# MAGIC-SCAN/adipose_tissue-unet

Measured on AMD Instinct MI355X. Metric: 1024^2 tiles/sec (train), higher is better.
Workload: dtype bf16; 1 GPU; unet_bn L5 base64 1024x1024x3 bf16 B=4/GPU (BASELINE configs[2]); preset=unet_bn, levels=5, tile=1024, batch_per_gpu=4, global_batch=4, parallelism=dp1

## Files before the change

### adipose_tissue-unet_amd/csrc/conv_fwd_halo.hip

```cpp
#include <type_traits>

#include "conv_common.h"

namespace {

__device__ __attribute__((aligned(256))) uint4 halo_zero_page[64];

constexpr int PH = 8, PW = 32;
constexpr int HH = PH + 2, HW = PW + 2;
constexpr int HROWS = HH * HW;
constexpr int ROWB = 128;

__device__ __forceinline__ int hswz(int r) { return r & 7; }

#define LDS_BAR()                                             \
  do {                                                        \
    asm volatile("s_waitcnt lgkmcnt(0)" ::: "memory");        \
    __builtin_amdgcn_s_barrier();                             \
    asm volatile("" ::: "memory");                            \
  } while (0)

#define HALO_BAR()                         \
  do {                                     \
    asm volatile("" ::: "memory");         \
    __builtin_amdgcn_s_barrier();          \
    asm volatile("" ::: "memory");         \
  } while (0)

template <int WN, int KS, int TPS, int NHB>
constexpr int halo_lds() {
  constexpr int NTH = 4 * WN * KS * 64;
  constexpr int GH = (HROWS * 8 + NTH - 1) / NTH;
  return NHB * (GH * NTH / 8) * ROWB + 3 * TPS * WN * 64 * ROWB;
}

template <int WN, int KS, int TPS, int NHB, bool BNR>
__global__ __launch_bounds__(4 * WN * KS * 64, (halo_lds<WN, KS, TPS, NHB>() <= 81920 ? 2 : 1))
void igemm_fwd_halo_kernel(FwdArgs a) {
  constexpr int NTH = 4 * WN * KS * 64;
  constexpr int BN = WN * 64;
  constexpr int SPC = (9 + TPS - 1) / TPS;
  constexpr int GH = (HROWS * 8 + NTH - 1) / NTH;
  constexpr int HROWS_PAD = GH * NTH / 8;
  constexpr int HBUF = HROWS_PAD * ROWB;
  constexpr int GB1 = BN * 8 / NTH;
  static_assert(GB1 * NTH == BN * 8, "weight slot must split evenly");
  constexpr int GB = GB1 * TPS;
  constexpr int WTAP = BN * ROWB;
  constexpr int WSLOT = TPS * WTAP;
  constexpr int OFF_W = NHB * HBUF;
  constexpr int LT = BN + 4;
  constexpr int EPI = PH * PW * LT * 4;
  constexpr int SMEM = (OFF_W + 3 * WSLOT > EPI) ? OFF_W + 3 * WSLOT : EPI;
  __shared__ __attribute__((aligned(1024))) unsigned char smem[SMEM];

  const int tid = threadIdx.x, lane = tid & 63;
  const int wave = __builtin_amdgcn_readfirstlane(tid >> 6);
  const int wm = wave % 4, wn = (wave / 4) % WN, kh = wave / (4 * WN);
  const int tx_n = a.Wo / PW, ty_n = a.Ho / PH;
  const int lin = xcd_remap(blockIdx.x, a.nblocks);
  const int tn = lin % a.ntile_n;
  int rest = lin / a.ntile_n;
  const int px = rest % tx_n; rest /= tx_n;
  const int py = rest % ty_n;
  const int img = rest / ty_n;
  const int y0 = py * PH, x0 = px * PW, n0 = tn * BN;
  const int Cin_s = a.CAs + a.CBs;
  const int nchunk = Cin_s / 64, nsteps = nchunk * SPC;
  const int Wrows = (a.Nout + 63) / 64 * 64;
  const bf16* srcA = reinterpret_cast<const bf16*>(a.srcA);
  const bf16* srcB = reinterpret_cast<const bf16*>(a.srcB);

  int hoff[GH], hcol[GH];
#pragma unroll
  for (int i = 0; i < GH; ++i) {
    const int idx = i * NTH + tid;
    const int hr = idx >> 3, pos = idx & 7;
    hcol[i] = 8 * (pos ^ hswz(hr));
    const int gy = y0 - 1 + hr / HW, gx = x0 - 1 + hr % HW;
    hoff[i] = (hr < HROWS && gy >= 0 && gy < a.Hs && gx >= 0 && gx < a.Ws) ? (img * a.Hs + gy) * a.Ws + gx : -1;
  }
  const bf16* wp[GB1];
#pragma unroll
  for (int i = 0; i < GB1; ++i) {
    const int idx = i * NTH + tid;
    const int q = idx >> 3, pos = idx & 7;
    wp[i] = (n0 + q < Wrows) ? reinterpret_cast<const bf16*>(a.W) + (size_t)(n0 + q) * a.Kpad + 8 * (pos ^ swz(q))
                             : nullptr;
  }

  auto issue_halo = [&](int c, int buf) {
    const int ci = c * 64;
    const bf16* base = ci < a.CAs ? srcA + ci : srcB + (ci - a.CAs);
    const int cs = ci < a.CAs ? a.CAs : a.CBs;
    unsigned char* dst = smem + buf * HBUF + wave * 8 * ROWB;
#pragma unroll
    for (int i = 0; i < GH; ++i) {
      const void* p = hoff[i] >= 0 ? (const void*)(base + (size_t)hoff[i] * cs + hcol[i]) : (const void*)halo_zero_page;
      __builtin_amdgcn_global_load_lds(p, (lds_void*)(dst + i * (NTH / 8) * ROWB), 16, 0, 0);
    }
  };
  auto issue_w = [&](int s) {
    const int c = s / SPC, j = s - SPC * c;
#pragma unroll
    for (int u = 0; u < TPS; ++u) {
      const int t = j * TPS + u;
      const int k = t * Cin_s + c * 64;
      unsigned char* dst = smem + OFF_W + (s % 3) * WSLOT + u * WTAP + wave * 8 * ROWB;
#pragma unroll
      for (int i = 0; i < GB1; ++i) {
        const void* p = (wp[i] && t < 9) ? (const void*)(wp[i] + k) : (const void*)halo_zero_page;
        __builtin_amdgcn_global_load_lds(p, (lds_void*)(dst + i * (NTH / 8) * ROWB), 16, 0, 0);
      }
    }
  };

  f32x4 acc[4][4];
#pragma unroll
  for (int i = 0; i < 4; ++i)
#pragma unroll
    for (int j = 0; j < 4; ++j) acc[i][j] = f32x4{0.f, 0.f, 0.f, 0.f};

  const int r16 = lane & 15, h4 = lane >> 4;
  issue_halo(0, 0);
  issue_w(0);
  if (nsteps > 1) {
    issue_w(1);
    asm volatile("s_waitcnt vmcnt(%0)" ::"n"(GB) : "memory");
  } else {
    asm volatile("s_waitcnt vmcnt(0)" ::: "memory");
  }
  HALO_BAR();

  for (int s = 0; s < nsteps; ++s) {
    const int c = s / SPC, j = s - SPC * c;
    const bool nh = NHB == 2 && j == 0 && c + 1 < nchunk;
    if (nh) issue_halo(c + 1, (c + 1) & 1);
    const bool nw = s + 2 < nsteps;
    if (nw) issue_w(s + 2);
    const unsigned char* H = smem + (NHB == 2 ? (c & 1) : 0) * HBUF;
#pragma unroll
    for (int u = 0; u < TPS; ++u) {
    const int t = j * TPS + u;
    if (t >= 9) break;
    const int dy = t / 3, dx = t - 3 * dy;
    const unsigned char* Wt = smem + OFF_W + (s % 3) * WSLOT + u * WTAP;
#pragma unroll
    for (int kq = 0; kq < 2 / KS; ++kq) {
      const int ck = 4 * (KS == 2 ? kh : kq) + h4;
      bf16x8 fb[4], fa[4];
#pragma unroll
      for (int nf = 0; nf < 4; ++nf) {
        const int q = wn * 64 + nf * 16 + r16;
        fb[nf] = *reinterpret_cast<const bf16x8*>(Wt + q * ROWB + ((ck ^ swz(q)) << 4));
      }
#pragma unroll
      for (int mf = 0; mf < 4; ++mf) {
        const int prow = 2 * wm + (mf >> 1), pcol = (mf & 1) * 16 + r16;
        const int hr = (prow + dy) * HW + pcol + dx;
        fa[mf] = *reinterpret_cast<const bf16x8*>(H + hr * ROWB + ((ck ^ hswz(hr)) << 4));
      }
#pragma unroll
      for (int mf = 0; mf < 4; ++mf)
#pragma unroll
        for (int nf = 0; nf < 4; ++nf)
          acc[mf][nf] = __builtin_amdgcn_mfma_f32_16x16x32_bf16(fa[mf], fb[nf], acc[mf][nf], 0, 0, 0);
    }
    }
    if (nw) {
      if (nh) asm volatile("s_waitcnt vmcnt(%0)" ::"n"(GB + GH) : "memory");
      else asm volatile("s_waitcnt vmcnt(%0)" ::"n"(GB) : "memory");
    } else {
      asm volatile("s_waitcnt vmcnt(0)" ::: "memory");
    }
    HALO_BAR();
  }

  float* tile = reinterpret_cast<float*>(smem);
  const int col = lane & 15, rq = (lane >> 4) * 4;
#pragma unroll
  for (int part = 0; part < KS; ++part) {
    if (kh == part) {
#pragma unroll
      for (int mf = 0; mf < 4; ++mf)
#pragma unroll
        for (int nf = 0; nf < 4; ++nf)
#pragma unroll
          for (int r = 0; r < 4; ++r) {
            const int p = (2 * wm + (mf >> 1)) * PW + (mf & 1) * 16 + rq + r;
            float* e = tile + p * LT + wn * 64 + nf * 16 + col;
            *e = part == 0 ? acc[mf][nf][r] : *e + acc[mf][nf][r];
          }
    }
    ADP_LDS_BARRIER();
  }
  float bs[8], bq[8];
#pragma unroll
  for (int j = 0; j < 8; ++j) { bs[j] = 0.f; bq[j] = 0.f; }
  for (int pr = 0; pr < PH; ++pr) {
    const int m0 = (img * a.Ho + y0 + pr) * a.Wo + x0;
    if constexpr (BNR) epi_rows_bnr<NTH, BN>(a, tile + pr * PW * LT, PW, m0, n0, tid, bs, bq);
    else epi_rows<NTH, BN>(a, tile + pr * PW * LT, PW, m0, n0, tid, bs, bq);
  }
  if (a.bn_sum || a.bnr_z) epi_bn_flush<NTH, BN>(a, tile, n0, tid, bs, bq);
}

#ifndef HALOP_VALU_PER_MFMA
#define HALOP_VALU_PER_MFMA 8
#endif
template <int I, int N, typename F>
__device__ __forceinline__ void halop_static_for(F&& f) {
  if constexpr (I < N) {
    f(std::integral_constant<int, I>{});
    halop_static_for<I + 1, N>(f);
  }
}
template <bool BNR, int NCH, int BN, bool PIPE, int EPI_, bool WIDE = false, bool DYN = false, bool SWP = false>
__global__ __launch_bounds__(512, 1) void igemm_fwd_halop_kernel(FwdArgs a) {
  constexpr bool BNL = EPI_ == 6;
  constexpr int EPI = BNL ? 1 : EPI_;
  static_assert(!BNL || (!BNR && !DYN && !SWP && NCH == 1), "BN-on-load: one-chunk static-list forward launches");
  static_assert(!BNR || EPI == 0, "the BN-backward reduction launch stores the plain product");
  static_assert(EPI < 4 || !PIPE, "mask / addend quads, the dropout hash and two accumulator sets: registers");
  constexpr int NTH = 512, NF = BN / 16;
  constexpr int HCH = NCH * HROWS * 8;
  constexpr int GH = (HCH + NTH - 1) / NTH;
  static_assert(!BNL || GH <= 6, "BN-on-load: at most six halo chunks per thread");
  constexpr int HBUF = HCH * 16;
  constexpr int GW = 9 * NCH * BN * 8 / NTH;
  constexpr int WTAP = NCH * BN * ROWB;
  constexpr int OFF_W = HBUF, OFF_C = OFF_W + 9 * WTAP;
  constexpr int OFF_S = OFF_C + 5 * BN * 4 + 16;
  constexpr int SMEM = OFF_S + (BNL ? 2 * NCH * 64 * 4 : 0);
  static_assert(GW * NTH == 9 * NCH * BN * 8, "weights must split evenly");
  static_assert(SMEM <= 160 * 1024, "LDS");
  typedef __bf16 bf16x4 __attribute__((ext_vector_type(4)));
  typedef unsigned int v2u32_h __attribute__((ext_vector_type(2)));
  typedef unsigned int v4u32_h __attribute__((ext_vector_type(4)));
  __shared__ __attribute__((aligned(1024))) unsigned char smem[SMEM];

  const int tid = threadIdx.x, lane = tid & 63;
  const int wave = __builtin_amdgcn_readfirstlane(tid >> 6);
  prio_static<ADP_PRIO_FWD>(wave);
  const int tx_n = a.Wo / PW, ty_n = a.Ho / PH;
  const int T = a.nblocks, G = gridDim.x;
  const int lin = xcd_remap(blockIdx.x, G);
  constexpr bool dyn = DYN;
  const bool full = dyn && a.claim_full;
  const int nt = dyn ? 0 : (lin < T ? (T - lin + G - 1) / G : 0);
  if (!dyn && nt == 0) return;
  const int Wrows = (a.Nout + 63) / 64 * 64;
  const int NT = a.ntile_n;
  const int nh = lin % NT, n0 = BN * nh;
  const bool second = a.out_mode == 2 && n0 >= a.split_c;
  bf16* obase = reinterpret_cast<bf16*>(second ? a.out2 : a.out);
  const int ostride = second ? a.out2_stride : a.out_stride;
  const int ocol0 = second ? n0 - a.split_c : n0;
  const int nlim = a.out_mode == 2 && !second ? a.split_c : a.Nout;
  const int Cin_s = a.CAs + a.CBs;

  int* ring = reinterpret_cast<int*>(smem + OFF_C + 5 * BN * 4);
  const int npatch = T / NT;
  const int CH = dyn ? a.claim_chunk : 1, nsup = (npatch + CH - 1) / CH;
  auto sup_id = [&](int sidx) -> int {
    const int v = full ? claim_ring_read(ring + (sidx & 3))
                       : sidx < 2 ? lin / NT + sidx * (G / NT) : 2 * (G / NT) + claim_ring_read(ring + (sidx & 3));
    return v < nsup ? v : -1;
  };
  auto tile_id = [&](int k) -> int {
    if (!dyn) return k < nt ? lin / NT + k * (G / NT) : -1;
    const int v = sup_id(k / CH);
    const int t = v * CH + k % CH;
    return v >= 0 && t < npatch ? t : -1;
  };
  if (full) {
    if (tid == 0) {
      const int r = claim_next2(a.claim + nh);
      ring[0] = r;
      ring[1] = r + 1;
    }
    __syncthreads();
  }
  if (dyn && tile_id(0) < 0) {
    if (tid == 0) claim_block_done(a.claim, NT, G);
    return;
  }
  auto tile_origin = [&](int t, int& img, int& y0, int& x0) {
    const int px = t % tx_n, r = t / tx_n;
    y0 = (r % ty_n) * PH;
    img = r / ty_n;
    x0 = px * PW;
  };
  auto halo_src = [&](int img, int y0, int x0, int i) -> const uint4* {
    const int idx = i * NTH + tid;
    const int cc = NCH == 1 ? 0 : (idx >= HROWS * 8 ? 1 : 0), hr = (idx - cc * HROWS * 8) >> 3;
    const int hy = hr / HW, hx = hr - hy * HW;
    const int gy = y0 + hy - 1, gx = x0 + hx - 1, us = a.up >> 1;
    const bool ok = (i < GH - 1 || idx < HCH) && (unsigned)gy < (unsigned)(a.Hs << us) && (unsigned)gx < (unsigned)(a.Ws << us);
    if (!ok) return nullptr;
    const bool inA = cc * 64 < a.CAs;
    const bf16* src = reinterpret_cast<const bf16*>(inA ? a.srcA : a.srcB);
    const int cs = inA ? a.CAs : a.CBs;
    return reinterpret_cast<const uint4*>(src + (size_t)((img * a.Hs + (gy >> us)) * a.Ws + (gx >> us)) * cs +
                                          (inA ? cc * 64 : cc * 64 - a.CAs) + 8 * ((tid & 7) ^ hswz(hr)));
  };

  const float* sS = reinterpret_cast<const float*>(smem + OFF_S);
  const bool act_w = BNL && n0 == 0 && a.act_out != nullptr && !(ADP_DBG(a) & 4096);
  const __amdgpu_buffer_rsrc_t rsA = __builtin_amdgcn_make_buffer_rsrc(
      a.act_out, 0, act_w ? a.Nimg * a.Hs * a.Ws * a.CAs * 2 : 0, 0x00020000);
  auto bnl = [&](uint4 v, int img, int y0, int x0, int i) -> uint4 {
    const int idx = i * NTH + tid;
    const int cc = NCH == 1 ? 0 : (idx >= HROWS * 8 ? 1 : 0), hr = (idx - cc * HROWS * 8) >> 3;
    const int hy = hr / HW, hx = hr - hy * HW;
    const int gy = y0 + hy - 1, gx = x0 + hx - 1;
    const bool inimg = (unsigned)gy < (unsigned)a.Hs && (unsigned)gx < (unsigned)a.Ws;
    const int c0 = cc * 64 + 8 * ((tid & 7) ^ hswz(hr));
    Grp<bf16> g;
    g.v = v;
    bf16* e = reinterpret_cast<bf16*>(&g.v);
#pragma unroll
    for (int hv = 0; hv < 2; ++hv) {
      const float4 q = *reinterpret_cast<const float4*>(sS + c0 + 4 * hv);
      const float4 r = *reinterpret_cast<const float4*>(sS + NCH * 64 + c0 + 4 * hv);
      e[4 * hv + 0] = (bf16)fmaxf(fmaf((float)e[4 * hv + 0], q.x, r.x), 0.f);
      e[4 * hv + 1] = (bf16)fmaxf(fmaf((float)e[4 * hv + 1], q.y, r.y), 0.f);
      e[4 * hv + 2] = (bf16)fmaxf(fmaf((float)e[4 * hv + 2], q.z, r.z), 0.f);
      e[4 * hv + 3] = (bf16)fmaxf(fmaf((float)e[4 * hv + 3], q.w, r.w), 0.f);
    }
    const bool wr = inimg && hy >= 1 && hy <= PH && hx >= 1 && hx <= PW;
    const unsigned off = wr ? (unsigned)((((img * a.Hs + gy) * a.Ws + gx) * a.CAs + c0) * 2) : 0x80000000u;
    if (act_w) __builtin_amdgcn_raw_buffer_store_b128(__builtin_bit_cast(v4u32_h, g.v), rsA, off, 0, 0);
    return inimg ? g.v : v;
  };

#pragma unroll
  for (int i = 0; i < GW; ++i) {
    const int idx = i * NTH + tid;
    const int tc = idx / (BN * 8), rem = idx - tc * BN * 8;
    const int t = tc / NCH, cc = tc - t * NCH;
    const int q = rem >> 3, pos = rem & 7;
    const void* p = n0 + q < Wrows
                        ? (const void*)(reinterpret_cast<const bf16*>(a.W) + (size_t)(n0 + q) * a.Kpad + t * Cin_s + cc * 64 +
                                        8 * (pos ^ swz(q)))
                        : (const void*)halo_zero_page;
    __builtin_amdgcn_global_load_lds(p, (lds_void*)(smem + OFF_W + (size_t)(i * NTH + wave * 64) * 16), 16, 0, 0);
  }
  int img0, y00, x00;
  tile_origin(tile_id(0), img0, y00, x00);
#pragma unroll
  for (int i = 0; i < GH; ++i) {
    if (i * NTH + tid < HCH) {
      const uint4* p = halo_src(img0, y00, x00, i);
      __builtin_amdgcn_global_load_lds(p ? (const void*)p : (const void*)halo_zero_page,
                                       (lds_void*)(smem + (size_t)(i * NTH + wave * 64) * 16), 16, 0, 0);
    }
  }
  float* cst = reinterpret_cast<float*>(smem + OFF_C);
  if (tid < BN) {
    const int c = n0 + tid;
    const bool v = c < a.Nout;
    cst[tid] = (!BNR && a.bias && v) ? a.bias[c] : 0.f;
    cst[BN + tid] = (BNR && v) ? a.bnr_sc[c] : 0.f;
    cst[2 * BN + tid] = (BNR && v) ? a.bnr_sh[c] : 0.f;
    cst[3 * BN + tid] = (BNR && v) ? -a.bnr_mean[c] * a.bnr_invstd[c] : 0.f;
    cst[4 * BN + tid] = (BNR && v) ? a.bnr_invstd[c] : 0.f;
  }
  if constexpr (BNL) {
    float* sw = reinterpret_cast<float*>(smem + OFF_S);
    if (tid < NCH * 64) {
      sw[tid] = a.scA[tid];
      sw[NCH * 64 + tid] = a.shA[tid];
    }
  }
  asm volatile("s_waitcnt vmcnt(0)" ::: "memory");
  __syncthreads();
  if constexpr (BNL) {
#pragma unroll
    for (int i = 0; i < GH; ++i)
      if (i * NTH + tid < HCH) {
        uint4* q = reinterpret_cast<uint4*>(smem + (size_t)(i * NTH + tid) * 16);
        *q = bnl(*q, img0, y00, x00, i);
      }
    __syncthreads();
  }

  const int r16 = lane & 15, h4 = lane >> 4;
  constexpr bool stats = BNR || EPI == 1 || EPI == 3;
  float s1[NF][4], s2[NF][4];
#pragma unroll
  for (int nf = 0; nf < NF; ++nf)
#pragma unroll
    for (int i = 0; i < 4; ++i) { s1[nf][i] = 0.f; s2[nf][i] = 0.f; }

  const __amdgpu_buffer_rsrc_t rsO =
      __builtin_amdgcn_make_buffer_rsrc((void*)obase, 0, a.M * ostride * 2, 0x00020000);
  const __amdgpu_buffer_rsrc_t rsZ = __builtin_amdgcn_make_buffer_rsrc(
      (void*)(BNR ? a.bnr_z : a.out), 0, BNR ? a.M * a.bnr_zs * 2 : 0, 0x00020000);
  const void* mptr = second ? a.mask2 : a.mask;
  const int mstr = second ? a.mask2_stride : a.mask_stride;
  const float mscale = second ? a.mask2_scale : a.mask_scale;
  const bool has_mask = EPI == 4 && mptr != nullptr, has_add = EPI == 4 && !second && a.addend != nullptr;
  const __amdgpu_buffer_rsrc_t rsM =
      __builtin_amdgcn_make_buffer_rsrc((void*)mptr, 0, has_mask ? a.M * mstr * 2 : 0, 0x00020000);
  const __amdgpu_buffer_rsrc_t rsD =
      __builtin_amdgcn_make_buffer_rsrc((void*)a.addend, 0, has_add ? a.M * a.addend_stride * 2 : 0, 0x00020000);
  auto load_q = [&](__amdgpu_buffer_rsrc_t rs, int str, int col0, int mrow_, uint2 (&zr)[2][NF]) {
#pragma unroll
    for (int mf = 0; mf < 2; ++mf)
#pragma unroll
      for (int nf = 0; nf < NF; ++nf) {
        const int c0 = nf * 16 + 4 * h4;
        const unsigned off = n0 + c0 < nlim ? (unsigned)(((mrow_ + mf * 16 + r16) * str + col0 + c0) * 2) : 0x80000000u;
        zr[mf][nf] = __builtin_bit_cast(uint2, __builtin_amdgcn_raw_buffer_load_b64(rs, off, 0, 0));
      }
  };
  auto load_z = [&](int mrow_, uint2 (&zr)[2][NF]) {
    if (ADP_DBG(a) & 8192) {
#pragma unroll
      for (int mf = 0; mf < 2; ++mf)
#pragma unroll
        for (int nf = 0; nf < NF; ++nf) zr[mf][nf] = uint2{0u, 0u};
      return;
    }
    load_q(rsZ, a.bnr_zs, n0, mrow_, zr);
  };
  auto epi_vals = [&](int mf, int nf, const f32x4& av, uint2 zv, int mrow_, uint2 dv = uint2{0u, 0u}) -> bf16x4 {
    const int c0 = nf * 16 + 4 * h4;
    const float4 cb = *reinterpret_cast<const float4*>(cst + c0);
    const int m = mrow_ + mf * 16 + r16;
    float v[4] = {av[0] + cb.x, av[1] + cb.y, av[2] + cb.z, av[3] + cb.w};
    if constexpr (EPI == 4) {
      const bf16x4 dd = __builtin_bit_cast(bf16x4, dv), mm = __builtin_bit_cast(bf16x4, zv);
#pragma unroll
      for (int i = 0; i < 4; ++i) {
        if (has_add) v[i] += (float)dd[i];
        if (has_mask) v[i] = (float)mm[i] > 0.f ? v[i] * mscale : 0.f;
      }
    }
    if constexpr (EPI == 5) {
      const float ks = 1.f / (1.f - a.drop_rate);
#pragma unroll
      for (int i = 0; i < 4; ++i) {
        const float u = adp_uniform(a.drop_seed, (uint64_t)m * (uint64_t)a.Nout + (n0 + c0 + i));
        v[i] = u >= a.drop_rate ? fmaxf(v[i], 0.f) * ks : 0.f;
      }
    }
    bf16x4 o;
#pragma unroll
    for (int i = 0; i < 4; ++i) {
      if constexpr (EPI == 2 || EPI == 3) v[i] = fmaxf(v[i], 0.f);
      o[i] = (bf16)v[i];
    }
    if constexpr (BNR) {
      if (ADP_DBG(a) & 16384) return o;
      const float4 sc = *reinterpret_cast<const float4*>(cst + BN + c0);
      const float4 sh = *reinterpret_cast<const float4*>(cst + 2 * BN + c0);
      const float4 nm = *reinterpret_cast<const float4*>(cst + 3 * BN + c0);
      const float4 is = *reinterpret_cast<const float4*>(cst + 4 * BN + c0);
      const float scv[4] = {sc.x, sc.y, sc.z, sc.w}, shv[4] = {sh.x, sh.y, sh.z, sh.w};
      const float nmv[4] = {nm.x, nm.y, nm.z, nm.w}, isv[4] = {is.x, is.y, is.z, is.w};
      bf16x4 zz = __builtin_bit_cast(bf16x4, zv);
#pragma unroll
      for (int i = 0; i < 4; ++i) {
        const float g = (float)o[i], zf = (float)zz[i];
        const float db = fmaf(zf, scv[i], shv[i]) > 0.f ? g : 0.f;
        s1[nf][i] += db;
        s2[nf][i] = fmaf(db, fmaf(zf, isv[i], nmv[i]), s2[nf][i]);
      }
    } else if constexpr (EPI == 1 || EPI == 3) {
#pragma unroll
      for (int i = 0; i < 4; ++i) {
        s1[nf][i] += v[i];
        s2[nf][i] = fmaf(v[i], v[i], s2[nf][i]);
      }
    }
    return o;
  };
  auto epi_unit = [&](int mf, int nf, const f32x4& av, uint2 zv, int mrow_, uint2 dv = uint2{0u, 0u}) {
    const bf16x4 o = epi_vals(mf, nf, av, zv, mrow_, dv);
    const int c0 = nf * 16 + 4 * h4, m = mrow_ + mf * 16 + r16;
    const unsigned off = n0 + c0 < nlim ? (unsigned)((m * ostride + ocol0 + c0) * 2) : 0x80000000u;
    __builtin_amdgcn_raw_buffer_store_b64(__builtin_bit_cast(v2u32_h, o), rsO, off, 0, 0);
  };
  auto epi_join = [&](int mf, int nf, v2u32_h o0, v2u32_h o1, int mrow_) {
    const auto e0 = __builtin_amdgcn_permlane16_swap(o0.x, o1.x, false, false);
    const auto e1 = __builtin_amdgcn_permlane16_swap(o0.y, o1.y, false, false);
    const v4u32_h st = {e0[0], e1[0], e0[1], e1[1]};
    const int cw = 16 * (nf + (h4 & 1)) + 8 * (h4 >> 1), m = mrow_ + mf * 16 + r16;
    const unsigned off = n0 + cw < nlim ? (unsigned)((m * ostride + ocol0 + cw) * 2) : 0x80000000u;
    __builtin_amdgcn_raw_buffer_store_b128(st, rsO, off, 0, 0);
  };
  auto epi_pair = [&](int mf, int nf, const f32x4& av0, const f32x4& av1, uint2 zv0, uint2 zv1, int mrow_,
                      uint2 dv0 = uint2{0u, 0u}, uint2 dv1 = uint2{0u, 0u}) {
    const v2u32_h o0 = __builtin_bit_cast(v2u32_h, epi_vals(mf, nf, av0, zv0, mrow_, dv0));
    const v2u32_h o1 = __builtin_bit_cast(v2u32_h, epi_vals(mf, nf + 1, av1, zv1, mrow_, dv1));
    epi_join(mf, nf, o0, o1, mrow_);
  };
  v2u32_h pend = {0u, 0u};
  auto epi_all = [&](const f32x4 (&av)[2][NF], const uint2 (&zv)[2][NF], int mrow_, const uint2 (&dv)[EPI == 4 ? 2 : 1][NF]) {
    if constexpr (WIDE) {
#pragma unroll
      for (int nf = 0; nf < NF; nf += 2)
#pragma unroll
        for (int mf = 0; mf < 2; ++mf)
          epi_pair(mf, nf, av[mf][nf], av[mf][nf + 1], zv[mf][nf], zv[mf][nf + 1], mrow_, dv[EPI == 4 ? mf : 0][nf],
                   dv[EPI == 4 ? mf : 0][nf + 1]);
    } else {
#pragma unroll
      for (int nf = 0; nf < NF; ++nf)
#pragma unroll
        for (int mf = 0; mf < 2; ++mf) epi_unit(mf, nf, av[mf][nf], zv[mf][nf], mrow_, dv[EPI == 4 ? mf : 0][nf]);
    }
  };

  f32x4 acc[2][NF], accp[2][NF];
  uint2 zreg[2][NF], dreg[EPI == 4 ? 2 : 1][NF];
  int mrowp = 0;
  auto load_halo = [&](int t, uint4 (&hr)[GH]) {
    int img1, y01, x01;
    tile_origin(t, img1, y01, x01);
    const bool nohalo = (ADP_DBG(a) & 1024) != 0;
#pragma unroll
    for (int i = 0; i < GH; ++i) {
      const uint4* p = nohalo ? nullptr : halo_src(img1, y01, x01, i);
      hr[i] = p ? *p : make_uint4(0, 0, 0, 0);
    }
  };
  auto run_tile = [&](int k, int tk, auto with_prev, uint4 (&hreg)[GH]) -> int {
    constexpr bool EPI_PREV = decltype(with_prev)::value;
    if constexpr (!DYN) tk = tile_id(k);
    const int tn = tile_id(k + 1);
    const bool more = tn >= 0;
    const bool claim_now = dyn && k % CH == 0 && more && sup_id(k / CH + 1) >= 0;
    int claimed = 0;
    if (claim_now && tid == 0) claimed = __hip_atomic_fetch_add(a.claim + nh, 1, __ATOMIC_RELAXED, __HIP_MEMORY_SCOPE_AGENT);
    int img, y0, x0;
    tile_origin(tk, img, y0, x0);
    const int mrow = (img * a.Ho + y0 + wave) * a.Wo + x0;
    if constexpr (BNR) load_z(EPI_PREV ? mrowp : mrow, zreg);
    if constexpr (EPI == 4) {
      if (has_mask) load_q(rsM, mstr, ocol0, mrow, zreg);
      if (has_add) load_q(rsD, a.addend_stride, ocol0, mrow, dreg);
    }
    if (more) load_halo(DYN ? tn : tile_id(k + 1), hreg);
    int img1 = 0, y01 = 0, x01 = 0;
    if constexpr (BNL) {
      if (more) tile_origin(tn, img1, y01, x01);
    }
#pragma unroll
    for (int i = 0; i < 2; ++i)
#pragma unroll
      for (int j = 0; j < NF; ++j) acc[i][j] = f32x4{0.f, 0.f, 0.f, 0.f};
    if constexpr (SWP) {
      constexpr int NS = 18 * NCH;
      bf16x8 FB[2][NF], FA[2][2];
      auto ldf = [&](auto sc, bf16x8 (&fb)[NF], bf16x8 (&fa)[2]) {
        constexpr int st = decltype(sc)::value, t = st / (2 * NCH), cc = (st >> 1) % NCH, kq = st & 1;
        constexpr int dy = t / 3, dx = t - 3 * dy;
        const unsigned char* Wt = smem + OFF_W + t * WTAP + cc * BN * ROWB;
        const unsigned char* Hc = smem + cc * HROWS * ROWB;
        const int ck = 4 * kq + h4;
#pragma unroll
        for (int nf = 0; nf < NF; ++nf) {
          const int q = nf * 16 + r16;
          fb[nf] = *reinterpret_cast<const bf16x8*>(Wt + q * ROWB + ((ck ^ swz(q)) << 4));
        }
#pragma unroll
        for (int mf = 0; mf < 2; ++mf) {
          const int hr = (wave + dy) * HW + mf * 16 + r16 + dx;
          fa[mf] = *reinterpret_cast<const bf16x8*>(Hc + hr * ROWB + ((ck ^ hswz(hr)) << 4));
        }
      };
      ldf(std::integral_constant<int, 0>{}, FB[0], FA[0]);
      halop_static_for<0, NS>([&](auto sc) {
        constexpr int st = decltype(sc)::value, t = st / (2 * NCH), cc = (st >> 1) % NCH, kq = st & 1;
        if constexpr (st + 1 < NS) ldf(std::integral_constant<int, st + 1>{}, FB[(st + 1) & 1], FA[(st + 1) & 1]);
        __builtin_amdgcn_sched_barrier(0);
        const bf16x8(&fb)[NF] = FB[st & 1];
        const bf16x8(&fa)[2] = FA[st & 1];
        constexpr bool with_unit = EPI_PREV && cc == 0 && kq == 0 && t >= 1 && t - 1 < 2 * NF;
        if constexpr (with_unit) {
          constexpr int u = t - 1;
          if constexpr (WIDE) {
            constexpr int p = u >> 1, mf = p & 1, nf = 2 * (p >> 1);
            if constexpr ((u & 1) == 0) {
              pend = __builtin_bit_cast(v2u32_h, epi_vals(mf, nf, accp[mf][nf], zreg[mf][nf], mrowp));
            } else {
              epi_join(mf, nf, pend, __builtin_bit_cast(v2u32_h, epi_vals(mf, nf + 1, accp[mf][nf + 1],
                                                                          zreg[mf][nf + 1], mrowp)), mrowp);
            }
          } else {
            epi_unit(u & 1, u >> 1, accp[u & 1][u >> 1], zreg[u & 1][u >> 1], mrowp);
          }
        }
        if constexpr (!with_unit) prio_hi<ADP_PRIO_FWD>();
#pragma unroll
        for (int mf = 0; mf < 2; ++mf)
#pragma unroll
          for (int nf = 0; nf < NF; ++nf)
            acc[mf][nf] = __builtin_amdgcn_mfma_f32_16x16x32_bf16(fb[nf], fa[mf], acc[mf][nf], 0, 0, 0);
        if constexpr (!with_unit) prio_lo<ADP_PRIO_FWD>();
        if constexpr (with_unit) {
#pragma unroll
          for (int i = 0; i < 2 * NF; ++i) {
            __builtin_amdgcn_sched_group_barrier(0x008, 1, 0);
            __builtin_amdgcn_sched_group_barrier(0x002, HALOP_VALU_PER_MFMA, 0);
          }
        }
      });
    }
#pragma unroll
    for (int t = 0; t < (SWP ? 0 : 9); ++t) {
      const int dy = t / 3, dx = t - 3 * dy;
#pragma unroll
      for (int cc = 0; cc < NCH; ++cc) {
        const unsigned char* Wt = smem + OFF_W + t * WTAP + cc * BN * ROWB;
        const unsigned char* Hc = smem + cc * HROWS * ROWB;
#pragma unroll
        for (int kq = 0; kq < 2; ++kq) {
          const int ck = 4 * kq + h4;
          bf16x8 fb[NF], fa[2];
#pragma unroll
          for (int nf = 0; nf < NF; ++nf) {
            const int q = nf * 16 + r16;
            fb[nf] = *reinterpret_cast<const bf16x8*>(Wt + q * ROWB + ((ck ^ swz(q)) << 4));
          }
#pragma unroll
          for (int mf = 0; mf < 2; ++mf) {
            const int hr = (wave + dy) * HW + mf * 16 + r16 + dx;
            fa[mf] = *reinterpret_cast<const bf16x8*>(Hc + hr * ROWB + ((ck ^ hswz(hr)) << 4));
          }
          constexpr bool unit_here = EPI_PREV;
          const bool with_unit = unit_here && cc == 0 && kq == 0 && t >= 1 && t - 1 < 2 * NF;
          if (with_unit) {
            const int u = t - 1;
            if constexpr (WIDE) {
              const int p = u >> 1, mf = p & 1, nf = 2 * (p >> 1);
              if ((u & 1) == 0) {
                pend = __builtin_bit_cast(v2u32_h, epi_vals(mf, nf, accp[mf][nf], zreg[mf][nf], mrowp));
              } else {
                epi_join(mf, nf, pend, __builtin_bit_cast(v2u32_h, epi_vals(mf, nf + 1, accp[mf][nf + 1],
                                                                            zreg[mf][nf + 1], mrowp)), mrowp);
              }
            } else {
              const int mf = u & 1, nf = u >> 1;
              epi_unit(mf, nf, accp[mf][nf], zreg[mf][nf], mrowp);
            }
          }
          const bool with_apply = BNL && kq == 1 && t >= 3 && t - 3 < GH;
          if constexpr (BNL) {
            if (with_apply && more) hreg[t - 3] = bnl(hreg[t - 3], img1, y01, x01, t - 3);
          }
          if (!with_unit && !with_apply) prio_hi<ADP_PRIO_FWD>();
#pragma unroll
          for (int mf = 0; mf < 2; ++mf)
#pragma unroll
            for (int nf = 0; nf < NF; ++nf)
              acc[mf][nf] = __builtin_amdgcn_mfma_f32_16x16x32_bf16(fb[nf], fa[mf], acc[mf][nf], 0, 0, 0);
          if (!with_unit && !with_apply) prio_lo<ADP_PRIO_FWD>();
          if (with_unit || with_apply) {
#pragma unroll
            for (int i = 0; i < 2 * NF; ++i) {
              __builtin_amdgcn_sched_group_barrier(0x008, 1, 0);
              __builtin_amdgcn_sched_group_barrier(0x002, HALOP_VALU_PER_MFMA, 0);
            }
          }
        }
      }
    }
    if constexpr (PIPE) {
#pragma unroll
      for (int i = 0; i < 2; ++i)
#pragma unroll
        for (int j = 0; j < NF; ++j) accp[i][j] = acc[i][j];
      mrowp = mrow;
    } else {
      epi_all(acc, zreg, mrow, dreg);
    }
    if (more) {
      LDS_BAR();
#pragma unroll
      for (int i = 0; i < GH; ++i)
        if (i * NTH + tid < HCH) *reinterpret_cast<uint4*>(smem + (size_t)(i * NTH + tid) * 16) = hreg[i];
      if (claim_now && tid == 0) ring[(k / CH + 2) & 3] = claimed;
      LDS_BAR();
    }
    return DYN ? tn : tile_id(k + 1);
  };
  uint4 hA[GH];
  int tnext = run_tile(0, tile_id(0), std::false_type{}, hA);
  for (int k = 1; tnext >= 0; ++k) tnext = run_tile(k, tnext, std::integral_constant<bool, PIPE>{}, hA);
  if constexpr (PIPE) {
    if constexpr (BNR) load_z(mrowp, zreg);
    epi_all(accp, zreg, mrowp, dreg);
  }
  if (dyn && tid == 0) claim_block_done(a.claim, NT, G);
  if (!stats || (ADP_DBG(a) & 2)) return;
  double* d0 = a.stat + (size_t)((blockIdx.x * 8 + wave) & (adp::STAT_REPL - 1)) * 2 * adp::STAT_CMAX;
#pragma unroll
  for (int nf = 0; nf < NF; ++nf)
#pragma unroll
    for (int i = 0; i < 4; ++i) {
      const float x = row16_sum(s1[nf][i]), y = row16_sum(s2[nf][i]);
      const int c = n0 + nf * 16 + 4 * h4 + i;
      if (r16 == 0 && c < a.Nout) {
        atomicAdd(d0 + c, (double)x);
        atomicAdd(d0 + adp::STAT_CMAX + c, (double)y);
      }
    }
}

#undef HALO_BAR
#undef LDS_BAR

template <int WN, int KS, int TPS, int NHB>
void launch_halo(FwdArgs& a, hipStream_t s) {
  constexpr int BN = WN * 64;
  a.ntile_n = (a.Nout + BN - 1) / BN;
  a.nblocks = a.Nimg * (a.Ho / PH) * (a.Wo / PW) * a.ntile_n;
  adp::set_kernel("igemm_fwd_halo_kernel<%d, %d, %d, %d, %s>", WN, KS, TPS, NHB, a.bnr_z ? "true" : "false");
  const dim3 g(a.nblocks), b(4 * WN * KS * 64);
  if (a.bnr_z) hipLaunchKernelGGL((igemm_fwd_halo_kernel<WN, KS, TPS, NHB, true>), g, b, 0, s, a);
  else hipLaunchKernelGGL((igemm_fwd_halo_kernel<WN, KS, TPS, NHB, false>), g, b, 0, s, a);
}

}

namespace adp {
int launch_fwd_halo(FwdArgs& a, hipStream_t s) {
  const int mode = option("fwd_halo", 1);
  if (mode == 0) return 0;
  const int Cin_s = a.CAs + a.CBs;
  const bool bnl = a.scA != nullptr;
  if (bnl && !(a.act_out && a.CBs == 0 && a.up == 1 && a.CAs == 64 && a.bn_sum && !a.bnr_z &&
               !a.relu && !a.bias && option("halop_bnl", 1)))
    return 0;
  if (a.scB || a.kh != 3 || a.kw != 3 || a.dil != 1 || a.pad != 1 || a.stride != 1 || (a.up != 1 && a.up != 2) ||
      a.Ho != a.Hs * a.up || a.Wo != a.Ws * a.up || a.Ho % PH != 0 || a.Wo % PW != 0 || a.CAs % 64 != 0 || a.CBs % 64 != 0 ||
      a.K != 9 * Cin_s || a.Kpad != a.K || a.Nout > 128)
    return 0;
  if (a.bnr_z && (a.out_mode != 0 || a.bias || a.relu || a.drop_rate > 0.f || a.accum || a.bn_sum)) return 0;
  const bool one_chunk = Cin_s == 64;
  const bool plain = !a.addend && !a.mask && !a.mask2 && !a.accum && a.drop_rate == 0.f && a.out_stride % 8 == 0;
  const bool dropepi = a.drop_rate > 0.f && a.relu && !a.addend && !a.mask && !a.mask2 && !a.accum && !a.bn_sum &&
                       !a.bnr_z && a.out_mode == 0 && a.out_stride % 8 == 0 && option("halop_dropout", 1);
  const bool maskepi = (a.addend || a.mask || a.mask2) && !a.accum && a.drop_rate == 0.f && !a.bnr_z && !a.bn_sum && !a.relu && !a.bias &&
                       a.out_stride % 8 == 0 && (!a.mask || a.mask_stride % 4 == 0) &&
                       (!a.mask2 || a.mask2_stride % 4 == 0) && (!a.addend || a.addend_stride % 4 == 0) &&
                       (size_t)a.M * std::max(std::max(a.mask ? a.mask_stride : 0, a.mask2 ? a.mask2_stride : 0),
                                              a.addend ? a.addend_stride : 0) * 2 < ((size_t)1 << 31) &&
                       option("halop_mask", 1);
  int bn = 0;
  if (one_chunk && (a.Nout <= 64 || a.Nout == 128)) bn = 64;
  else if (Cin_s == 128 && (a.Nout == 64 || a.Nout == 128) && option("halo_persist2", 1)) bn = 32;
  const int nt_n = bn ? (a.Nout + bn - 1) / bn : 1;
  const bool split_ok = a.out_mode == 2 && bn && a.split_c > 0 && a.split_c % bn == 0 && a.split_c < a.Nout &&
                        (!a.mask2 || maskepi) && a.out2_stride % 8 == 0 && (a.Nout - a.split_c) % bn == 0;
  const size_t lim = (size_t)1 << 31;
  const bool fits = (size_t)a.M * a.out_stride * 2 < lim && (!a.out2 || (size_t)a.M * a.out2_stride * 2 < lim) &&
                    (!a.bnr_z || (size_t)a.M * a.bnr_zs * 2 < lim);
  if (bn && (plain || maskepi || dropepi) && fits && (a.out_mode == 0 || split_ok) && option("halo_persist", 1) &&
      (a.up == 1 || !a.bnr_z)) {
    const int tiles = a.Nimg * (a.Ho / PH) * (a.Wo / PW) * nt_n;
    a.ntile_n = nt_n;
    a.nblocks = tiles;
    int grid = std::max(1, std::min(tiles, option("halo_persist_grid", 256)));
    grid -= grid % nt_n;
    if (grid == 0) grid = nt_n;
    const bool bnr = a.bnr_z != nullptr;
    const int pm = option("halop_pipe", 1);
    const int swm = option("halop_swp", 2);
    const bool swp_req = !bnr && !dropepi && (swm == 1 || (swm == 2 && !one_chunk));
    const bool pipe = !swp_req && !bnr && !maskepi && !dropepi && (pm == 2 || (pm == 1 && one_chunk));
    const int epi = bnr ? 0 : dropepi ? 5 : maskepi ? 4 : (a.bn_sum ? 1 : 0) + (a.relu ? 2 : 0);
    const int wm = option("halop_wide", 3);
    const bool wide = !bnr && (wm == 2 || (wm == 1 && !pipe) || (wm == 3 && !(pipe && (epi == 1 || epi == 3)))) &&
                      a.Nout % 8 == 0 && (a.out_mode != 2 || a.split_c % 8 == 0);
    a.claim = option("halop_claim", option("dp_claim", 0)) && nt_n + 1 <= CLAIM_INTS && !(bnr && one_chunk) && !(pipe && (epi == 1 || epi == 3))
                  ? claim_slot() : nullptr;
    a.claim_chunk = std::max(1, option("halop_claim_chunk", 4));
    a.claim_full = 0;
    if (a.claim) {
      const int nsup = (tiles / nt_n + a.claim_chunk - 1) / a.claim_chunk;
      grid = std::max(nt_n, std::min(grid, nsup * nt_n));
      a.claim_full = option("claim_full", 0) && nsup >= 4 * (grid / nt_n);
    }
    if (bnl) a.claim = nullptr;
    const bool dyn = a.claim != nullptr;
    const bool swp = !dyn && swp_req;
    if (bnl) {
      if (one_chunk && a.Nout <= 64 && pipe && !wide && !swp && epi == 1) {
        adp::set_kernel("igemm_fwd_halop_kernel<false, 1, 64, true, 6, false, false, false>");
        hipLaunchKernelGGL((igemm_fwd_halop_kernel<false, 1, 64, true, 6, false, false, false>), dim3(grid), dim3(512), 0,
                           s, a);
        return 1;
      }
      return 0;
    }
    adp::set_kernel("igemm_fwd_halop_kernel<%s, %d, %d, %s, %d, %s, %s, %s>", bnr ? "true" : "false", one_chunk ? 1 : 2, bn,
                    pipe ? "true" : "false", epi, wide ? "true" : "false", dyn ? "true" : "false", swp ? "true" : "false");
#define HALOP_LAUNCH_WD(NCH_, BN_, W_, D_, P_)                                                                   \
  do {                                                                                                      \
    if (bnr) hipLaunchKernelGGL((igemm_fwd_halop_kernel<true, NCH_, BN_, false, 0, false, D_, P_>), dim3(grid), dim3(512), 0, s, a); \
    else if (epi == 4) hipLaunchKernelGGL((igemm_fwd_halop_kernel<false, NCH_, BN_, false, 4, W_, D_, P_>), dim3(grid), dim3(512), 0, s, a); \
    else if (epi == 5) hipLaunchKernelGGL((igemm_fwd_halop_kernel<false, NCH_, BN_, false, 5, W_, D_, P_>), dim3(grid), dim3(512), 0, s, a); \
    else if (pipe) {                                                                                        \
      if (epi == 1) hipLaunchKernelGGL((igemm_fwd_halop_kernel<false, NCH_, BN_, true, 1, W_, D_, P_>), dim3(grid), dim3(512), 0, s, a); \
      else if (epi == 2) hipLaunchKernelGGL((igemm_fwd_halop_kernel<false, NCH_, BN_, true, 2, W_, D_, P_>), dim3(grid), dim3(512), 0, s, a); \
      else if (epi == 3) hipLaunchKernelGGL((igemm_fwd_halop_kernel<false, NCH_, BN_, true, 3, W_, D_, P_>), dim3(grid), dim3(512), 0, s, a); \
      else hipLaunchKernelGGL((igemm_fwd_halop_kernel<false, NCH_, BN_, true, 0, W_, D_, P_>), dim3(grid), dim3(512), 0, s, a); \
    } else {                                                                                                \
      if (epi == 1) hipLaunchKernelGGL((igemm_fwd_halop_kernel<false, NCH_, BN_, false, 1, W_, D_, P_>), dim3(grid), dim3(512), 0, s, a); \
      else if (epi == 2) hipLaunchKernelGGL((igemm_fwd_halop_kernel<false, NCH_, BN_, false, 2, W_, D_, P_>), dim3(grid), dim3(512), 0, s, a); \
      else if (epi == 3) hipLaunchKernelGGL((igemm_fwd_halop_kernel<false, NCH_, BN_, false, 3, W_, D_, P_>), dim3(grid), dim3(512), 0, s, a); \
      else hipLaunchKernelGGL((igemm_fwd_halop_kernel<false, NCH_, BN_, false, 0, W_, D_, P_>), dim3(grid), dim3(512), 0, s, a); \
    }                                                                                                       \
  } while (0)
#define HALOP_LAUNCH_SWP(NCH_, BN_, W_)                                                                         \
  do {                                                                                                      \
    if (epi == 4) hipLaunchKernelGGL((igemm_fwd_halop_kernel<false, NCH_, BN_, false, 4, W_, false, true>), dim3(grid), dim3(512), 0, s, a); \
    else if (epi == 1) hipLaunchKernelGGL((igemm_fwd_halop_kernel<false, NCH_, BN_, false, 1, W_, false, true>), dim3(grid), dim3(512), 0, s, a); \
    else if (epi == 2) hipLaunchKernelGGL((igemm_fwd_halop_kernel<false, NCH_, BN_, false, 2, W_, false, true>), dim3(grid), dim3(512), 0, s, a); \
    else if (epi == 3) hipLaunchKernelGGL((igemm_fwd_halop_kernel<false, NCH_, BN_, false, 3, W_, false, true>), dim3(grid), dim3(512), 0, s, a); \
    else hipLaunchKernelGGL((igemm_fwd_halop_kernel<false, NCH_, BN_, false, 0, W_, false, true>), dim3(grid), dim3(512), 0, s, a); \
  } while (0)
#define HALOP_LAUNCH_W(NCH_, BN_, W_)                          \
  do {                                                         \
    if (dyn) HALOP_LAUNCH_WD(NCH_, BN_, W_, true, false);      \
    else if (swp) HALOP_LAUNCH_SWP(NCH_, BN_, W_);              \
    else HALOP_LAUNCH_WD(NCH_, BN_, W_, false, false);         \
  } while (0)
#define HALOP_LAUNCH(NCH_, BN_)                  \
  do {                                           \
    if (wide) HALOP_LAUNCH_W(NCH_, BN_, true);   \
    else HALOP_LAUNCH_W(NCH_, BN_, false);       \
  } while (0)
    if (one_chunk) HALOP_LAUNCH(1, 64);
    else HALOP_LAUNCH(2, 32);
#undef HALOP_LAUNCH_W
#undef HALOP_LAUNCH_WD
#undef HALOP_LAUNCH_SWP
#undef HALOP_LAUNCH
    return 1;
  }
  if (bnl) return 0;
  if (a.Nout == 128 && Cin_s > 128 && !a.bnr_z && plain && a.out_mode != 1 && option("halo_defer_tap64p", 1))
    return 0;
  if (a.up != 1) return 0;
  if (a.Nout <= 64) {
    if (one_chunk && mode != 2) launch_halo<1, 2, 1, 1>(a, s);
    else launch_halo<1, 2, 2, 2>(a, s);
  } else {
    if (one_chunk && mode != 2) launch_halo<2, 1, 1, 1>(a, s);
    else launch_halo<2, 1, 1, 2>(a, s);
  }
  return 1;
}
}
```

Measured before the change: 184.3 tiles/s.

## Stage BN-backward z tile into LDS via async loads; precompute LDS fragment offsets

```diff
diff --git a/adipose_tissue-unet_amd/csrc/conv_fwd_halo.hip b/adipose_tissue-unet_amd/csrc/conv_fwd_halo.hip
--- a/adipose_tissue-unet_amd/csrc/conv_fwd_halo.hip
+++ b/adipose_tissue-unet_amd/csrc/conv_fwd_halo.hip
@@ -218,8 +218,10 @@
 template <bool BNR, int NCH, int BN, bool PIPE, int EPI_, bool WIDE = false, bool DYN = false, bool SWP = false>
 __global__ __launch_bounds__(512, 1) void igemm_fwd_halop_kernel(FwdArgs a) {
   constexpr bool BNL = EPI_ == 6;
-  constexpr int EPI = BNL ? 1 : EPI_;
+  constexpr bool ZL = EPI_ == 7;
+  constexpr int EPI = BNL ? 1 : ZL ? 0 : EPI_;
   static_assert(!BNL || (!BNR && !DYN && !SWP && NCH == 1), "BN-on-load: one-chunk static-list forward launches");
+  static_assert(!ZL || (BNR && !PIPE && !DYN && NCH == 1), "LDS-staged z: the one-chunk static-list BNR launch");
   static_assert(!BNR || EPI == 0, "the BN-backward reduction launch stores the plain product");
   static_assert(EPI < 4 || !PIPE, "mask / addend quads, the dropout hash and two accumulator sets: registers");
   constexpr int NTH = 512, NF = BN / 16;
@@ -231,7 +233,9 @@
   constexpr int WTAP = NCH * BN * ROWB;
   constexpr int OFF_W = HBUF, OFF_C = OFF_W + 9 * WTAP;
   constexpr int OFF_S = OFF_C + 5 * BN * 4 + 16;
-  constexpr int SMEM = OFF_S + (BNL ? 2 * NCH * 64 * 4 : 0);
+  constexpr int OFF_Z = (OFF_S + 1023) / 1024 * 1024;
+  constexpr int ZROW = PW * BN * 2;
+  constexpr int SMEM = ZL ? OFF_Z + PH * ZROW : OFF_S + (BNL ? 2 * NCH * 64 * 4 : 0);
   static_assert(GW * NTH == 9 * NCH * BN * 8, "weights must split evenly");
   static_assert(SMEM <= 160 * 1024, "LDS");
   typedef __bf16 bf16x4 __attribute__((ext_vector_type(4)));
@@ -291,8 +295,11 @@
     img = r / ty_n;
     x0 = px * PW;
   };
+  constexpr bool LEAN = EPI_ == 7;
   auto halo_src = [&](int img, int y0, int x0, int i) -> const uint4* {
-    const int idx = i * NTH + tid;
+    int ht = tid;
+    if constexpr (LEAN) asm volatile("" : "+v"(ht));
+    const int idx = i * NTH + ht;
     const int cc = NCH == 1 ? 0 : (idx >= HROWS * 8 ? 1 : 0), hr = (idx - cc * HROWS * 8) >> 3;
     const int hy = hr / HW, hx = hr - hy * HW;
     const int gy = y0 + hy - 1, gx = x0 + hx - 1, us = a.up >> 1;
@@ -302,7 +309,7 @@
     const bf16* src = reinterpret_cast<const bf16*>(inA ? a.srcA : a.srcB);
     const int cs = inA ? a.CAs : a.CBs;
     return reinterpret_cast<const uint4*>(src + (size_t)((img * a.Hs + (gy >> us)) * a.Ws + (gx >> us)) * cs +
-                                          (inA ? cc * 64 : cc * 64 - a.CAs) + 8 * ((tid & 7) ^ hswz(hr)));
+                                          (inA ? cc * 64 : cc * 64 - a.CAs) + 8 * ((ht & 7) ^ hswz(hr)));
   };
 
   const float* sS = reinterpret_cast<const float*>(smem + OFF_S);
@@ -425,6 +432,14 @@
     }
     load_q(rsZ, a.bnr_zs, n0, mrow_, zr);
   };
+  auto issue_z = [&](int mrow_, int nf) {
+    if (ADP_DBG(a) & 8192) return;
+    const bf16* src = reinterpret_cast<const bf16*>(a.bnr_z) + (size_t)(mrow_ + (lane >> 1)) * a.bnr_zs + n0 + 16 * nf + 8 * (lane & 1);
+    __builtin_amdgcn_global_load_lds((const void*)src, (lds_void*)(smem + OFF_Z + wave * ZROW + nf * 1024), 16, 0, 0);
+  };
+  auto z_lds = [&](int mf, int nf) -> uint2 {
+    return *reinterpret_cast<const uint2*>(smem + OFF_Z + wave * ZROW + nf * 1024 + (mf * 16 + r16) * 32 + 8 * h4);
+  };
   auto epi_vals = [&](int mf, int nf, const f32x4& av, uint2 zv, int mrow_, uint2 dv = uint2{0u, 0u}) -> bf16x4 {
     const int c0 = nf * 16 + 4 * h4;
     const float4 cb = *reinterpret_cast<const float4*>(cst + c0);
@@ -503,17 +518,32 @@
 #pragma unroll
       for (int nf = 0; nf < NF; nf += 2)
 #pragma unroll
-        for (int mf = 0; mf < 2; ++mf)
-          epi_pair(mf, nf, av[mf][nf], av[mf][nf + 1], zv[mf][nf], zv[mf][nf + 1], mrow_, dv[EPI == 4 ? mf : 0][nf],
-                   dv[EPI == 4 ? mf : 0][nf + 1]);
+        for (int mf = 0; mf < 2; ++mf) {
+          if constexpr (ZL) epi_pair(mf, nf, av[mf][nf], av[mf][nf + 1], z_lds(mf, nf), z_lds(mf, nf + 1), mrow_);
+          else epi_pair(mf, nf, av[mf][nf], av[mf][nf + 1], zv[mf][nf], zv[mf][nf + 1], mrow_, dv[EPI == 4 ? mf : 0][nf],
+                        dv[EPI == 4 ? mf : 0][nf + 1]);
+        }
     } else {
 #pragma unroll
       for (int nf = 0; nf < NF; ++nf)
 #pragma unroll
-        for (int mf = 0; mf < 2; ++mf) epi_unit(mf, nf, av[mf][nf], zv[mf][nf], mrow_, dv[EPI == 4 ? mf : 0][nf]);
-    }
-  };
-
+        for (int mf = 0; mf < 2; ++mf) {
+          if constexpr (ZL) epi_unit(mf, nf, av[mf][nf], z_lds(mf, nf), mrow_);
+          else epi_unit(mf, nf, av[mf][nf], zv[mf][nf], mrow_, dv[EPI == 4 ? mf : 0][nf]);
+        }
+    }
+  };
+
+  int hxa[7][2], wxa[2];
+  if constexpr (LEAN) {
+    const int hr0 = wave * HW + r16;
+#pragma unroll
+    for (int kq = 0; kq < 2; ++kq) {
+#pragma unroll
+      for (int k7 = 0; k7 < 7; ++k7) hxa[k7][kq] = hr0 * ROWB + (((4 * kq + h4) ^ hswz(hr0 + k7)) << 4);
+      wxa[kq] = r16 * ROWB + (((4 * kq + h4) ^ swz(r16)) << 4);
+    }
+  }
   f32x4 acc[2][NF], accp[2][NF];
   uint2 zreg[2][NF], dreg[EPI == 4 ? 2 : 1][NF];
   int mrowp = 0;
@@ -538,7 +568,11 @@
     int img, y0, x0;
     tile_origin(tk, img, y0, x0);
     const int mrow = (img * a.Ho + y0 + wave) * a.Wo + x0;
-    if constexpr (BNR) load_z(EPI_PREV ? mrowp : mrow, zreg);
+    if constexpr (ZL) {
+#pragma unroll
+      for (int nf = 0; nf < NF; ++nf) issue_z(mrow, nf);
+    }
+    else if constexpr (BNR) load_z(EPI_PREV ? mrowp : mrow, zreg);
     if constexpr (EPI == 4) {
       if (has_mask) load_q(rsM, mstr, ocol0, mrow, zreg);
       if (has_add) load_q(rsD, a.addend_stride, ocol0, mrow, dreg);
@@ -558,6 +592,16 @@
       auto ldf = [&](auto sc, bf16x8 (&fb)[NF], bf16x8 (&fa)[2]) {
         constexpr int st = decltype(sc)::value, t = st / (2 * NCH), cc = (st >> 1) % NCH, kq = st & 1;
         constexpr int dy = t / 3, dx = t - 3 * dy;
+        if constexpr (LEAN) {
+#pragma unroll
+          for (int nf = 0; nf < NF; ++nf)
+            fb[nf] = *reinterpret_cast<const bf16x8*>(smem + OFF_W + t * WTAP + cc * BN * ROWB + nf * 16 * ROWB + wxa[kq]);
+          halop_static_for<0, 2>([&](auto mfc) {
+            constexpr int mf = decltype(mfc)::value, K = dy * HW + mf * 16 + dx;
+            fa[mf] = *reinterpret_cast<const bf16x8*>(smem + cc * HROWS * ROWB + K * ROWB + hxa[K & 7][kq]);
+          });
+          return;
+        }
         const unsigned char* Wt = smem + OFF_W + t * WTAP + cc * BN * ROWB;
         const unsigned char* Hc = smem + cc * HROWS * ROWB;
         const int ck = 4 * kq + h4;
@@ -624,12 +668,15 @@
 #pragma unroll
           for (int nf = 0; nf < NF; ++nf) {
             const int q = nf * 16 + r16;
-            fb[nf] = *reinterpret_cast<const bf16x8*>(Wt + q * ROWB + ((ck ^ swz(q)) << 4));
+            if constexpr (LEAN) fb[nf] = *reinterpret_cast<const bf16x8*>(Wt + nf * 16 * ROWB + wxa[kq]);
+            else fb[nf] = *reinterpret_cast<const bf16x8*>(Wt + q * ROWB + ((ck ^ swz(q)) << 4));
           }
 #pragma unroll
           for (int mf = 0; mf < 2; ++mf) {
             const int hr = (wave + dy) * HW + mf * 16 + r16 + dx;
-            fa[mf] = *reinterpret_cast<const bf16x8*>(Hc + hr * ROWB + ((ck ^ hswz(hr)) << 4));
+            const int K = dy * HW + mf * 16 + dx;
+            if constexpr (LEAN) fa[mf] = *reinterpret_cast<const bf16x8*>(Hc + K * ROWB + hxa[K & 7][kq]);
+            else fa[mf] = *reinterpret_cast<const bf16x8*>(Hc + hr * ROWB + ((ck ^ hswz(hr)) << 4));
           }
           constexpr bool unit_here = EPI_PREV;
           const bool with_unit = unit_here && cc == 0 && kq == 0 && t >= 1 && t - 1 < 2 * NF;
@@ -676,6 +723,7 @@
         for (int j = 0; j < NF; ++j) accp[i][j] = acc[i][j];
       mrowp = mrow;
     } else {
+      if constexpr (ZL) asm volatile("s_waitcnt vmcnt(0)" ::: "memory");
       epi_all(acc, zreg, mrow, dreg);
     }
     if (more) {
@@ -771,12 +819,16 @@
     const bool bnr = a.bnr_z != nullptr;
     const int pm = option("halop_pipe", 1);
     const int swm = option("halop_swp", 2);
-    const bool swp_req = !bnr && !dropepi && (swm == 1 || (swm == 2 && !one_chunk));
+    const int zlm = bnr && one_chunk ? option("halop_bnr_lds", 1) : 0;
+    const bool zl = (zlm == 1 || zlm == 2 || zlm == 4) && a.Nout % 64 == 0 && a.bnr_zs % 8 == 0 &&
+                    (reinterpret_cast<uintptr_t>(a.bnr_z) & 15) == 0;
+    const bool swp_req = bnr ? zl && zlm != 2 : !dropepi && (swm == 1 || (swm == 2 && !one_chunk));
     const bool pipe = !swp_req && !bnr && !maskepi && !dropepi && (pm == 2 || (pm == 1 && one_chunk));
-    const int epi = bnr ? 0 : dropepi ? 5 : maskepi ? 4 : (a.bn_sum ? 1 : 0) + (a.relu ? 2 : 0);
+    const int epi = bnr ? (zl ? 7 : 0) : dropepi ? 5 : maskepi ? 4 : (a.bn_sum ? 1 : 0) + (a.relu ? 2 : 0);
     const int wm = option("halop_wide", 3);
-    const bool wide = !bnr && (wm == 2 || (wm == 1 && !pipe) || (wm == 3 && !(pipe && (epi == 1 || epi == 3)))) &&
-                      a.Nout % 8 == 0 && (a.out_mode != 2 || a.split_c % 8 == 0);
+    const bool wide = bnr ? zl && zlm == 1
+                          : (wm == 2 || (wm == 1 && !pipe) || (wm == 3 && !(pipe && (epi == 1 || epi == 3)))) &&
+                                a.Nout % 8 == 0 && (a.out_mode != 2 || a.split_c % 8 == 0);
     a.claim = option("halop_claim", option("dp_claim", 0)) && nt_n + 1 <= CLAIM_INTS && !(bnr && one_chunk) && !(pipe && (epi == 1 || epi == 3))
                   ? claim_slot() : nullptr;
     a.claim_chunk = std::max(1, option("halop_claim_chunk", 4));
@@ -800,6 +852,12 @@
     }
     adp::set_kernel("igemm_fwd_halop_kernel<%s, %d, %d, %s, %d, %s, %s, %s>", bnr ? "true" : "false", one_chunk ? 1 : 2, bn,
                     pipe ? "true" : "false", epi, wide ? "true" : "false", dyn ? "true" : "false", swp ? "true" : "false");
+    if (zl) {
+      if (wide) hipLaunchKernelGGL((igemm_fwd_halop_kernel<true, 1, 64, false, 7, true, false, true>), dim3(grid), dim3(512), 0, s, a);
+      else if (swp) hipLaunchKernelGGL((igemm_fwd_halop_kernel<true, 1, 64, false, 7, false, false, true>), dim3(grid), dim3(512), 0, s, a);
+      else hipLaunchKernelGGL((igemm_fwd_halop_kernel<true, 1, 64, false, 7, false, false, false>), dim3(grid), dim3(512), 0, s, a);
+      return 1;
+    }
 #define HALOP_LAUNCH_WD(NCH_, BN_, W_, D_, P_)                                                                   \
   do {                                                                                                      \
     if (bnr) hipLaunchKernelGGL((igemm_fwd_halop_kernel<true, NCH_, BN_, false, 0, false, D_, P_>), dim3(grid), dim3(512), 0, s, a); \
```

Result: no change. 184.5 tiles/s (median of 3 runs) (+0.1%).
